# bebop/poly

Measured on AMD Instinct MI355X. Metric: mash.Sketch k-mers hashed/s, higher is better.
Workload: dtype u32

## Files before the change

### poly_amd/csrc/mash_sketch.hip

```cpp
#include <hip/hip_runtime.h>

#include <algorithm>

#include "common.h"
#include "host_pipeline.h"
#include "multi_device.h"
#include <memory>
#include <string>
#include <vector>

#ifndef PH_WPE
#define PH_WPE 6
#endif
#ifndef PH_CAPK
#define PH_CAPK 12u
#endif
#ifndef PH_ABL
#define PH_ABL 0
#endif
#ifndef PH_SEL_ATOMIC
#define PH_SEL_ATOMIC 0
#endif
#ifndef PH_BS_WIN
#define PH_BS_WIN 4
#endif
#ifndef PH_BS_U
#define PH_BS_U 4
#endif
#ifndef PH_SLAB_SIG
#define PH_SLAB_SIG 6u
#endif
#ifndef PH_SLAB_CW
#define PH_SLAB_CW 6u
#endif
#ifndef PH_SLAB_CF
#define PH_SLAB_CF 0u
#endif
#ifndef PH_SLAB_WPE
#define PH_SLAB_WPE 8
#endif

namespace polyhip {
namespace k1 {

constexpr int THREADS = 256;
constexpr int WAVES = THREADS / 64;
#ifndef PH_WTW
#define PH_WTW 512
#endif
constexpr int WTW = PH_WTW;
constexpr int TW = WTW * WAVES;
constexpr int GROUPS = WTW / (4 * 64);
constexpr int NB = 2048;
constexpr uint32_t MARK0 = 0xFFFFFFFFu, MARK1 = 0u;
constexpr int GBATCH = 32;
constexpr uint32_t WL_POSITIONAL = 0x80000000u;
constexpr uint32_t C1 = 0xcc9e2d51u, C2 = 0x1b873593u;

__device__ __forceinline__ uint32_t rotl32(uint32_t x, int r) { return (x << r) | (x >> (32 - r)); }

__device__ __forceinline__ uint32_t premix(uint32_t k)
{
    k *= C1;
    k = rotl32(k, 15);
    k *= C2;
    return k;
}

__device__ __forceinline__ uint32_t chain(uint32_t h) { return rotl32(h, 13) * 5u + 0xe6546b64u; }

__device__ __forceinline__ uint32_t fmix32(uint32_t h)
{
    h ^= h >> 16;
    h *= 0x85ebca6bu;
    h ^= h >> 13;
    h *= 0xc2b2ae35u;
    h ^= h >> 16;
    return h;
}

__device__ __forceinline__ uint32_t funnel_bytes(uint32_t hi, uint32_t lo, uint32_t sh)
{
    return __builtin_amdgcn_alignbyte(hi, lo, sh);
}

__device__ __forceinline__ uint32_t wave_incl_scan(uint32_t v)
{
    v += (uint32_t)__builtin_amdgcn_update_dpp(0, (int)v, 0x111, 0xF, 0xF, true);
    v += (uint32_t)__builtin_amdgcn_update_dpp(0, (int)v, 0x112, 0xF, 0xF, true);
    v += (uint32_t)__builtin_amdgcn_update_dpp(0, (int)v, 0x114, 0xF, 0xF, true);
    v += (uint32_t)__builtin_amdgcn_update_dpp(0, (int)v, 0x118, 0xF, 0xF, true);
    v += (uint32_t)__builtin_amdgcn_update_dpp(0, (int)v, 0x142, 0xA, 0xF, false);
    v += (uint32_t)__builtin_amdgcn_update_dpp(0, (int)v, 0x143, 0xC, 0xF, false);
    return v;
}

struct Smem {
    uint32_t *seqb;
    uint32_t *P;
    uint32_t *cand;
    uint32_t *binned;
    uint32_t *misc;
    uint32_t *lut;
    uint32_t *bins;
    uint32_t *biglist;
    uint32_t listcap;
};

constexpr uint32_t BIG_BIN = 32;
constexpr uint32_t BIG_LIST_CAP = 512;

template <class Bin, class Emit>
__device__ __attribute__((noinline)) void rank_big_bins(const uint32_t *__restrict__ binned, const Bin *__restrict__ bins,
                                              const uint32_t *__restrict__ biglist, uint32_t nbig, uint32_t s, Emit emit)
{
    const int lane = threadIdx.x & 63, wave = threadIdx.x >> 6;
    const uint64_t below = (1ull << lane) - 1ull;
    for (uint32_t q = wave; q < nbig; q += WAVES) {
        const uint32_t b = biglist[q];
        const uint32_t st = b ? bins[b - 1] : 0u, en = bins[b];
        uint32_t base = st, lastv = 0;
        bool first = true;
        while (base < s && base < en) {
            uint32_t m = 0xFFFFFFFFu;
            bool has = false;
            for (uint32_t x = st + lane; x < en; x += 64) {
                const uint32_t o = binned[x];
                if (first || o > lastv) {
                    m = min(m, o);
                    has = true;
                }
            }
            if (__ballot(has) == 0ull)
                break;
#pragma unroll
            for (int d = 32; d >= 1; d >>= 1)
                m = min(m, (uint32_t)__shfl_xor((int)m, d, 64));
            for (uint32_t x0 = st; x0 < en; x0 += 64) {
                const uint32_t x = x0 + lane;
                const bool eq = x < en && binned[x] == m;
                const uint64_t mask = __ballot(eq);
                const uint32_t pos = base + (uint32_t)__builtin_popcountll(mask & below);
                if (eq && pos < s)
                    emit(pos, m);
                base += (uint32_t)__builtin_popcountll(mask);
            }
            lastv = m;
            first = false;
        }
    }
}

template <class ForEach>
__device__ uint32_t bottom_s(const Smem &sm, uint32_t s, uint32_t tau, uint32_t binned_cap, bool keep_partial,
                             ForEach for_each)
{
    const int tid = threadIdx.x;
    uint32_t *bins = sm.P;
    const int sig = 32 - __builtin_clz(tau | 1u);
    const int shift = sig > 11 ? sig - 11 : 0;
    __syncthreads();
// ... 166 lines not shown
    const int tail = (int)(k & 3);
    const uint32_t tailmask = tail == 0 ? 0u : (0xFFFFFFFFu >> (32 - 8 * tail));

    {
        const int nq = (WTW >> 2) + nblk;
        for (int q = lane; q < (PH_ABL == 1 ? 0 : nq); q += 64) {
            const uint32_t d0 = seqb[q], d1 = seqb[q + 1];
            uint4 p;
            p.x = premix(d0);
            p.y = premix(funnel_bytes(d1, d0, 1));
            p.z = premix(funnel_bytes(d1, d0, 2));
            p.w = premix(funnel_bytes(d1, d0, 3));
            reinterpret_cast<uint4 *>(P)[q] = p;
        }
    }
    wave_sync();

    const uint4 *P4 = reinterpret_cast<const uint4 *>(P);
#pragma unroll
    for (int g = 0; g < GROUPS; ++g) {
        const int wq = lane + 64 * g;
        uint32_t h[4] = {0u, 0u, 0u, 0u};
        if (KS > 0) {
#pragma unroll
            for (int j = 0; j < (PH_ABL == 2 ? 1 : (KS >> 2)); ++j) {
                const uint4 p = P4[wq + j];
                h[0] = chain(h[0] ^ p.x);
                h[1] = chain(h[1] ^ p.y);
                h[2] = chain(h[2] ^ p.z);
                h[3] = chain(h[3] ^ p.w);
            }
        } else {
            for (int j = 0; j < nblk; ++j) {
                const uint4 p = P4[wq + j];
                h[0] = chain(h[0] ^ p.x);
                h[1] = chain(h[1] ^ p.y);
                h[2] = chain(h[2] ^ p.z);
                h[3] = chain(h[3] ^ p.w);
            }
        }
        if (PH_ABL == 3) {
        } else if (tail == 1) {
            const uint32_t tb = seqb[wq + nblk];
            h[0] ^= lut[tb & 0xFFu];
            h[1] ^= lut[(tb >> 8) & 0xFFu];
            h[2] ^= lut[(tb >> 16) & 0xFFu];
            h[3] ^= lut[tb >> 24];
        } else if (tail) {
            const uint32_t d0 = seqb[wq + nblk], d1 = seqb[wq + nblk + 1];
            h[0] ^= premix(d0 & tailmask) ^ k;
            h[1] ^= premix(funnel_bytes(d1, d0, 1) & tailmask) ^ k;
            h[2] ^= premix(funnel_bytes(d1, d0, 2) & tailmask) ^ k;
            h[3] ^= premix(funnel_bytes(d1, d0, 3) & tailmask) ^ k;
        } else {
#pragma unroll
            for (int c = 0; c < 4; ++c)
                h[c] ^= k;
        }
#pragma unroll
        for (int c = 0; c < 4; ++c)
            h[c] = PH_ABL == 3 ? h[c] : fmix32(h[c]);
        emit(4u * (uint32_t)wq, h);
    }
    wave_sync();
}

template <int KS, bool LOCKSTEP, class Before, class EmitFull, class EmitPart>
__device__ __forceinline__ void run_tiles(const Smem &sm, const uint32_t *__restrict__ gdw, uint32_t gsh,
                                          int64_t gbytes, int64_t nwin, uint32_t k, uint32_t n_seq_dw, uint32_t n_P_w,
                                          Before before, EmitFull emit_full, EmitPart emit_part)
{
    const int wave = threadIdx.x >> 6;
    uint32_t *seqb = sm.seqb + wave * n_seq_dw;
    uint32_t *P = sm.P + wave * n_P_w;
    const int64_t stage_bytes = (int64_t)n_seq_dw * 4 + 4;
    auto is_full = [&](int64_t t0) { return (nwin - t0) >= (int64_t)WTW && t0 + stage_bytes <= gbytes; };
    Stager<KS> st;
    const int64_t first = (int64_t)wave * WTW;
    if (first < nwin)
        st.load(gdw, gsh, gbytes, first, n_seq_dw, is_full(first));
    for (int64_t T0 = 0; T0 < nwin; T0 += TW) {
        if (LOCKSTEP)
            before(T0);
        const int64_t t0 = T0 + first;
        if (t0 >= nwin)
            continue;
        const bool full = is_full(t0);
        st.store(seqb, gdw, gsh, gbytes, t0, n_seq_dw, full);
        wave_sync();
        if (t0 + TW < nwin)
            st.load(gdw, gsh, gbytes, t0 + TW, n_seq_dw, is_full(t0 + TW));
        if (full) {
            tile_compute<KS>(seqb, P, sm.lut, k, [&](uint32_t w0, const uint32_t(&h)[4]) { emit_full(t0, w0, h, 4u); });
        } else {
            const uint32_t wl = (uint32_t)((nwin - t0) < (int64_t)WTW ? (nwin - t0) : (int64_t)WTW);
            tile_compute<KS>(seqb, P, sm.lut, k, [&](uint32_t w0, const uint32_t(&h)[4]) {
                emit_part(t0, w0, h, w0 >= wl ? 0u : (wl - w0 < 4u ? wl - w0 : 4u));
            });
        }
    }
}

__device__ __forceinline__ void append4(uint32_t *__restrict__ counter, uint32_t *__restrict__ cand, uint32_t cap,
                                        const uint32_t (&h)[4], uint32_t nvalid, uint32_t tau)
{
    bool a[4];
    uint64_t m[4];
    uint32_t cnt[4], total = 0;
#pragma unroll
    for (int c = 0; c < 4; ++c) {
        a[c] = (PH_ABL == 4 ? h[c] == 12345u : h[c] <= tau) && (uint32_t)c < nvalid;
        m[c] = __ballot(a[c]);
        cnt[c] = (uint32_t)__popcll(m[c]);
        total += cnt[c];
    }
    if (total == 0)
        return;
    uint32_t base = 0;
    if ((threadIdx.x & 63) == 0)
        base = atomicAdd(counter, total);
    base = __builtin_amdgcn_readfirstlane(base);
#pragma unroll
    for (int c = 0; c < 4; ++c) {
        if (a[c]) {
            const uint32_t idx = base + __builtin_amdgcn_mbcnt_hi((uint32_t)(m[c] >> 32),
                                                                  __builtin_amdgcn_mbcnt_lo((uint32_t)m[c], 0u));
            if (idx < cap)
                cand[idx] = h[c];
        }
        base += cnt[c];
    }
}

constexpr int BSU = PH_BS_U;
constexpr uint32_t BS_MARGIN = (PH_BS_WIN + 3u) & ~3u;
#define BS_SYNC()              \
    do {                       \
        if (PH_ABL != 21)      \
            __syncthreads();   \
    } while (0)
template <bool FIN>
__device__ void bottom_s_fast(const Smem &sm, uint32_t s, uint32_t tau, uint32_t C, uint32_t nbf_log2,
                              uint32_t *__restrict__ outp, const uint32_t *__restrict__ src, uint32_t first,
                              uint32_t step, uint32_t cnt)
{
    const int tid = threadIdx.x;
    auto fin = [](uint32_t h) { return FIN ? h ^ (h >> 16) : h; };
    uint32_t *bins = sm.bins;
    const uint16_t *bins16 = reinterpret_cast<const uint16_t *>(bins);
    const int sig = 32 - __builtin_clz(tau | 1u);
    const int shift = sig > (int)nbf_log2 ? sig - (int)nbf_log2 : 0;
    auto one = [](uint32_t b) { return 1u << ((b & 1u) << 4); };
    const bool wide = nbf_log2 == 11u;
    if (wide)
        reinterpret_cast<uint4 *>(bins)[tid] = make_uint4(0, 0, 0, 0);
    else
        reinterpret_cast<uint2 *>(bins)[tid] = make_uint2(0, 0);
    if (tid == 0)
        sm.misc[8] = 0;
    if (PH_BS_WIN) {
        if (tid < PH_BS_WIN)
            sm.binned[-1 - tid] = 0u;
        else if (tid < 2 * PH_BS_WIN)
            sm.binned[C + (uint32_t)tid - PH_BS_WIN] = 0xFFFFFFFFu;
    }
    BS_SYNC();
    for (uint32_t i0 = first; i0 < cnt; i0 += BSU * step) {
        uint32_t h[BSU];
#pragma unroll
        for (int u = 0; u < BSU; ++u)
            h[u] = i0 + u * step < cnt ? fin(src[i0 + u * step]) : 0u;
#pragma unroll
        for (int u = 0; u < BSU; ++u)
            if (i0 + u * step < cnt) {
                const uint32_t b = h[u] >> shift;
                atomicAdd(&bins[b >> 1], one(b));
            }
    }
    BS_SYNC();
    {
        uint32_t w[4];
        if (wide) {
            const uint4 t = reinterpret_cast<const uint4 *>(bins)[tid];
            w[0] = t.x, w[1] = t.y, w[2] = t.z, w[3] = t.w;
        } else {
            const uint2 t = reinterpret_cast<const uint2 *>(bins)[tid];
            w[0] = t.x, w[1] = t.y, w[2] = 0u, w[3] = 0u;
        }
        uint32_t c[8], sum = 0;
#pragma unroll
        for (int i = 0; i < 8; ++i) {
            c[i] = (w[i >> 1] >> (16 * (i & 1))) & 0xFFFFu;
            sum += c[i];
        }
        const uint32_t incl = wave_incl_scan(sum);
        if ((tid & 63) == 63)
            sm.misc[4 + (tid >> 6)] = incl;
        BS_SYNC();
        uint32_t run = incl - sum;
        for (int w8 = 0; w8 < (tid >> 6); ++w8)
            run += sm.misc[4 + w8];
        const uint32_t b0 = (uint32_t)tid << (wide ? 3 : 2);
#pragma unroll
        for (int i = 0; i < 4; ++i) {
            w[i] = run | ((run + c[2 * i]) << 16);
            run += c[2 * i] + c[2 * i + 1];
        }
        if (wide)
            reinterpret_cast<uint4 *>(bins)[tid] = make_uint4(w[0], w[1], w[2], w[3]);
        else
            reinterpret_cast<uint2 *>(bins)[tid] = make_uint2(w[0], w[1]);
        if (max(max(max(c[0], c[1]), max(c[2], c[3])), max(max(c[4], c[5]), max(c[6], c[7]))) > BIG_BIN) {
#pragma unroll
            for (int i = 0; i < 8; ++i)
                if (c[i] > BIG_BIN) {
                    const uint32_t slot = atomicAdd(&sm.misc[8], 1u);
                    if (slot < sm.listcap)
                        sm.biglist[slot] = b0 + (uint32_t)i;
                }
        }
    }
    BS_SYNC();
    for (uint32_t i0 = first; i0 < cnt; i0 += BSU * step) {
        uint32_t h[BSU], at[BSU];
#pragma unroll
        for (int u = 0; u < BSU; ++u)
            h[u] = i0 + u * step < cnt ? fin(src[i0 + u * step]) : 0u;
#pragma unroll
        for (int u = 0; u < BSU; ++u)
            if (i0 + u * step < cnt) {
                const uint32_t b = h[u] >> shift;
                at[u] = (atomicAdd(&bins[b >> 1], one(b)) >> ((b & 1u) << 4)) & 0xFFFFu;
            }
#pragma unroll
        for (int u = 0; u < BSU; ++u)
            if (i0 + u * step < cnt)
                sm.binned[at[u]] = h[u];
    }
    BS_SYNC();
    const uint32_t nbig = sm.misc[8];
    const bool by_waves = nbig <= sm.listcap;
    auto rank_in_bin = [&](uint32_t j, uint32_t hv) {
        const uint32_t b = hv >> shift;
        const uint32_t start = b ? bins16[b - 1] : 0u, end = bins16[b];
        if (start >= s || (by_waves && end - start > BIG_BIN))
            return;
        uint32_t pos = start;
        for (uint32_t x = start; x < end; ++x) {
            const uint32_t o = sm.binned[x];
            pos += (o < hv) || (o == hv && x < j);
        }
        if (pos < s)
            outp[pos] = hv;
    };
#if PH_BS_WIN
    if (PH_ABL != 22) {
        const uint32_t lim = 1u << shift;
        for (uint32_t j = tid; j < C; j += THREADS) {
            const uint32_t *__restrict__ w = sm.binned + j;
            const uint32_t hv = w[0];
            uint32_t pos = j;
            bool far;
            {
                uint32_t l[PH_BS_WIN], r[PH_BS_WIN];
#pragma unroll
                for (int d = 0; d < PH_BS_WIN; ++d) {
                    l[d] = w[-1 - d];
                    r[d] = w[1 + d];
                }
#pragma unroll
                for (int d = 0; d < PH_BS_WIN; ++d) {
                    pos -= l[d] > hv ? 1u : 0u;
                    pos += r[d] < hv ? 1u : 0u;
                }
                far = ((l[PH_BS_WIN - 1] ^ hv) < lim) | ((r[PH_BS_WIN - 1] ^ hv) < lim);
            }
            if (__builtin_expect(far, 0))
                rank_in_bin(j, hv);
            else if (pos < s)
                outp[pos] = hv;
        }
    }
#else
    for (uint32_t j = tid; j < C; j += THREADS)
        rank_in_bin(j, sm.binned[j]);
#endif
    if (by_waves && nbig)
        rank_big_bins(sm.binned, bins16, sm.biglist, nbig, s, [outp](uint32_t pos, uint32_t hv) { outp[pos] = hv; });
}

struct ReadView {
    const uint32_t *gdw;
    uint32_t gsh;
    int64_t gbytes, nwin;
};

__device__ __forceinline__ ReadView view(const uint8_t *__restrict__ seqs, const uint64_t *__restrict__ offs,
                                         uint64_t r, uint32_t k)
{
    ReadView v;
    const uint64_t o0 = offs[r], o1 = offs[r + 1];
    const int64_t n = (int64_t)(o1 - o0);
    v.nwin = n - (int64_t)k;
    v.gsh = (uint32_t)((uintptr_t)(seqs + o0) & 3);
    v.gdw = reinterpret_cast<const uint32_t *>(seqs + o0 - v.gsh);
    v.gbytes = n + v.gsh;
    return v;
}

template <int KS>
__global__ __launch_bounds__(THREADS) __attribute__((amdgpu_waves_per_eu(PH_WPE, 8))) void sketch_fast_kernel(const uint8_t *__restrict__ seqs,
                                                             const uint64_t *__restrict__ offs, uint64_t nseq,
                                                             uint32_t k_rt, uint32_t s, uint32_t *__restrict__ out,
                                                             uint32_t n_seq_dw, uint32_t n_P_w, uint32_t n_P,
                                                             uint32_t capf, uint32_t nbf_log2)
{
    extern __shared__ __attribute__((aligned(16))) uint32_t smem_raw[];
    Smem sm;
    sm.seqb = smem_raw;
    sm.P = sm.seqb + WAVES * n_seq_dw;
    sm.cand = sm.P + n_P;
    sm.binned = sm.cand + capf + BS_MARGIN;
    sm.misc = sm.binned + capf + BS_MARGIN;
    sm.lut = sm.misc + 16;
    sm.bins = sm.P;
    sm.biglist = sm.seqb;
    sm.listcap = BIG_LIST_CAP;

    const uint32_t k = KS > 0 ? (uint32_t)KS : k_rt;
    const int tid = threadIdx.x;
    sm.lut[tid] = premix((uint32_t)tid) ^ k;
    auto nothing = [](int64_t) {};

    for (uint64_t r = blockIdx.x; r < nseq; r += gridDim.x) {
        const ReadView rv = view(seqs, offs, r, k);
        if (rv.nwin <= 0)
            continue;
        uint32_t *__restrict__ outp = out + r * (uint64_t)s;

        if (rv.nwin < (int64_t)s) {
            __syncthreads();
            auto put = [&](int64_t t0, uint32_t w0, const uint32_t(&h)[4], uint32_t nvalid) {
#pragma unroll
                for (int c = 0; c < 4; ++c)
                    if ((uint32_t)c < nvalid)
                        outp[t0 + w0 + c] = h[c];
            };
            run_tiles<KS, false>(sm, rv.gdw, rv.gsh, rv.gbytes, rv.nwin, k, n_seq_dw, n_P_w, nothing, put, put);
            continue;
        }

        uint32_t tau0 = 0xFFFFFFFFu;
        {
            const uint64_t target = (uint64_t)s + 6ull * (uint64_t)__builtin_sqrtf((float)s) + 16ull;
            if ((int64_t)target < rv.nwin)
                tau0 = (uint32_t)((target << 32) / (uint64_t)rv.nwin);
        }
        bool ok = tau0 != 0xFFFFFFFFu || rv.nwin <= (int64_t)capf;
        __syncthreads();
        if (tid == 0)
            sm.misc[0] = 0;
        __syncthreads();
        uint32_t C = 0;
        if (ok) {
            auto keep = [&](int64_t, uint32_t, const uint32_t(&h)[4], uint32_t nvalid) {
                append4(&sm.misc[0], sm.cand, capf, h, nvalid, tau0);
            };
            run_tiles<KS, false>(sm, rv.gdw, rv.gsh, rv.gbytes, rv.nwin, k, n_seq_dw, n_P_w, nothing, keep, keep);
            __syncthreads();
            C = sm.misc[0];
            ok = C >= s && C <= capf;
        }
        if (ok) {
            if (PH_ABL == 5) {
                for (uint32_t i = tid; i < s; i += THREADS)
                    outp[i] = sm.cand[i];
            } else {
                bottom_s_fast<false>(sm, s, tau0, C, nbf_log2, outp, sm.cand, (uint32_t)tid, THREADS, C);
            }
        } else if (tid == 0) {
            outp[0] = MARK0;
            outp[1] = MARK1;
        }
    }
}

template <int KS> struct Slabs {
    static constexpr int NBLK = KS >> 2, TAIL = KS & 3;
    static constexpr int DUPD = NBLK + 2;
    const uint32_t *__restrict__ gdw;
    uint32_t gsh;
    uint32_t *__restrict__ seqb;
    uint32_t *__restrict__ P;
    const uint32_t *__restrict__ lut;
    int lane;

    uint32_t u_inside;
    uint32_t gb32;
    __device__ __forceinline__ void gload(uint32_t u, uint32_t &lo, uint32_t &hi) const
    {
        const uint32_t *__restrict__ slab = gdw + (uint64_t)u * 64;
        hi = 0u;
        if (__builtin_expect(u < u_inside, 1)) {
            lo = slab[lane];
            if (gsh)
                hi = slab[lane + 1];
        } else {
            const int left = (int)(gb32 - u * 256u);
            lo = lane * 4 < left ? slab[lane] : 0u;
            if (gsh)
                hi = (lane + 1) * 4 < left ? slab[lane + 1] : 0u;
        }
    }

    template <int PAR> __device__ __forceinline__ void stage(uint32_t lo, uint32_t hi) const
    {
        const uint32_t v = gsh ? funnel_bytes(hi, lo, gsh) : lo;
        seqb[1 + 64 * PAR + lane] = v;
        if (PAR == 0) {
            if (lane < DUPD)
                seqb[129 + lane] = v;
        } else if (lane == 63) {
            seqb[0] = v;
        }
    }

    template <int PAR> __device__ __forceinline__ void premix_unit() const
    {
        const uint32_t d0 = seqb[64 * PAR + lane], d1 = seqb[64 * PAR + lane + 1];
        uint4 p;
        p.x = premix(d0);
        p.y = premix(funnel_bytes(d1, d0, 1));
        p.z = premix(funnel_bytes(d1, d0, 2));
        p.w = premix(funnel_bytes(d1, d0, 3));
        uint4 *P4 = reinterpret_cast<uint4 *>(P);
        if (PAR == 0) {
            P4[(lane + 127) & 127] = p;
            if (lane >= 1 && lane <= NBLK)
                P4[127 + lane] = p;
        } else {
            P4[63 + lane] = p;
        }
    }

    template <int PAR> __device__ __forceinline__ void hash(uint32_t (&h)[4]) const
    {
        const uint4 *b = reinterpret_cast<const uint4 *>(P) + 64 * PAR + lane;
        h[0] = h[1] = h[2] = h[3] = 0u;
#pragma unroll
        for (int j = 0; j < (PH_ABL == 16 ? 1 : NBLK); ++j) {
            const uint4 p = b[j];
            h[0] = chain(h[0] ^ p.x);
            h[1] = chain(h[1] ^ p.y);
            h[2] = chain(h[2] ^ p.z);
            h[3] = chain(h[3] ^ p.w);
        }
        const uint32_t *t = seqb + 1 + 64 * PAR + lane + NBLK;
        if (TAIL == 1) {
            const uint32_t tb = t[0];
            uint32_t off[4];
            const uint32_t two = 2u;
            asm("v_lshlrev_b32_sdwa %0, %1, %2 dst_sel:DWORD dst_unused:UNUSED_PAD src0_sel:DWORD src1_sel:BYTE_0" : "=v"(off[0]) : "v"(two), "v"(tb));
            asm("v_lshlrev_b32_sdwa %0, %1, %2 dst_sel:DWORD dst_unused:UNUSED_PAD src0_sel:DWORD src1_sel:BYTE_1" : "=v"(off[1]) : "v"(two), "v"(tb));
            asm("v_lshlrev_b32_sdwa %0, %1, %2 dst_sel:DWORD dst_unused:UNUSED_PAD src0_sel:DWORD src1_sel:BYTE_2" : "=v"(off[2]) : "v"(two), "v"(tb));
            asm("v_lshlrev_b32_sdwa %0, %1, %2 dst_sel:DWORD dst_unused:UNUSED_PAD src0_sel:DWORD src1_sel:BYTE_3" : "=v"(off[3]) : "v"(two), "v"(tb));
#pragma unroll
            for (int c = 0; c < 4; ++c)
                h[c] ^= *reinterpret_cast<const __attribute__((address_space(3))) uint32_t *>((uintptr_t)off[c]);
        } else if (TAIL) {
            constexpr uint32_t tailmask = 0xFFFFFFFFu >> (32 - 8 * (TAIL ? TAIL : 1));
            const uint32_t d0 = t[0], d1 = t[1];
            h[0] ^= premix(d0 & tailmask) ^ (uint32_t)KS;
            h[1] ^= premix(funnel_bytes(d1, d0, 1) & tailmask) ^ (uint32_t)KS;
            h[2] ^= premix(funnel_bytes(d1, d0, 2) & tailmask) ^ (uint32_t)KS;
            h[3] ^= premix(funnel_bytes(d1, d0, 3) & tailmask) ^ (uint32_t)KS;
        } else {
#pragma unroll
            for (int c = 0; c < 4; ++c)
                h[c] ^= (uint32_t)KS;
        }
#pragma unroll
        for (int c = 0; c < 4; ++c) {
            uint32_t x = h[c];
            if (PH_ABL != 17) {
                x ^= x >> 16;
                x *= 0x85ebca6bu;
                x ^= x >> 13;
            }
            x *= 0xc2b2ae35u;
            h[c] = x;
        }
    }
};

template <bool PARTIAL>
__device__ __forceinline__ void append_own(uint32_t *__restrict__ seg, uint32_t capw, uint32_t &cnt, const uint32_t (&h)[4],
                                           uint32_t nvalid, uint32_t tauq)
{
    bool a[4];
    uint64_t m[4];
    uint32_t n[4], total = 0;
#pragma unroll
    for (int c = 0; c < 4; ++c) {
        a[c] = h[c] <= tauq && (!PARTIAL || (uint32_t)c < nvalid);
        m[c] = __ballot(a[c]);
        n[c] = (uint32_t)__popcll(m[c]);
        total += n[c];
    }
    uint32_t base = __builtin_amdgcn_readfirstlane(cnt);
    cnt = base + total;
#if PH_SEL_ATOMIC
    {
        uint32_t *ctr = seg + capw;
        uint32_t slot[4];
#pragma unroll
        for (int c = 0; c < 4; ++c)
            if (a[c])
                slot[c] = atomicInc(ctr, capw - 1u);
#pragma unroll
        for (int c = 0; c < 4; ++c)
            if (a[c])
                seg[slot[c]] = h[c];
        return;
    }
#endif
    if (cnt <= capw) {
#pragma unroll
        for (int c = 0; c < 4; ++c) {
            uint32_t *__restrict__ at = seg + base;
            if (a[c])
                at[__builtin_amdgcn_mbcnt_hi((uint32_t)(m[c] >> 32), __builtin_amdgcn_mbcnt_lo((uint32_t)m[c], 0u))] = h[c];
            base += n[c];
        }
    }
}

template <int KS>
__device__ __forceinline__ uint32_t run_slabs(const Smem &sm, const ReadView &rv, uint32_t n_seq_dw, uint32_t n_P_w,
                                              uint32_t *__restrict__ seg, uint32_t capw, uint32_t tauq)
{
    const int wave = __builtin_amdgcn_readfirstlane(threadIdx.x >> 6);
    Slabs<KS> S;
    S.gdw = rv.gdw;
    S.gsh = rv.gsh;
    S.seqb = sm.seqb + wave * n_seq_dw;
    S.P = sm.P + wave * n_P_w;
    S.lut = sm.lut;
    S.lane = threadIdx.x & 63;
    const uint32_t nslab = (uint32_t)((rv.nwin + 255) >> 8);
    const uint32_t spw = (nslab + WAVES - 1) / WAVES;
    const uint32_t a = (uint32_t)wave * spw, b = a + spw < nslab ? a + spw : nslab;
    S.u_inside = rv.gbytes >= 65 * 4 ? (uint32_t)(((rv.gbytes >> 2) - 65) >> 6) + 1u : 0u;
    S.gb32 = (uint32_t)rv.gbytes;
    const uint32_t nfull = (uint32_t)(rv.nwin >> 8), rem = (uint32_t)rv.nwin & 255u;
    uint32_t cnt = 0;
#if PH_SEL_ATOMIC
    capw -= 1u;
    if (S.lane == 0)
        seg[capw] = 0u;
#endif
    if (a >= b)
        return cnt;
    uint32_t l1, h1;
    S.gload(a, l1, h1);
    if (a & 1) {
        S.template stage<1>(l1, h1);
        wave_sync();
        S.gload(a + 1, l1, h1);
        S.template premix_unit<1>();
    } else {
        S.template stage<0>(l1, h1);
        wave_sync();
        S.gload(a + 1, l1, h1);
        S.template premix_unit<0>();
    }
    for (uint32_t i = a; i < b; ++i) {
        uint32_t h[4];
        if (i & 1) {
            S.template stage<0>(l1, h1);
            wave_sync();
            S.gload(i + 2, l1, h1);
            if (PH_ABL != 15)
                S.template premix_unit<0>();
            wave_sync();
            S.template hash<1>(h);
        } else {
            S.template stage<1>(l1, h1);
            wave_sync();
            S.gload(i + 2, l1, h1);
            if (PH_ABL != 15)
                S.template premix_unit<1>();
            wave_sync();
            S.template hash<0>(h);
        }
        if (PH_ABL == 11) {
            if ((h[0] ^ h[1] ^ h[2] ^ h[3]) == 0x12345u)
                seg[0] = h[0];
        } else if (__builtin_expect(i < nfull, 1)) {
            append_own<false>(seg, capw, cnt, h, 4u, tauq);
        } else {
            const int mine = (int)rem - 4 * S.lane;
            append_own<true>(seg, capw, cnt, h, mine <= 0 ? 0u : (mine < 4 ? (uint32_t)mine : 4u), tauq);
        }
        wave_sync();
    }
    return cnt;
}

template <int KS>
__global__ __launch_bounds__(THREADS) __attribute__((amdgpu_waves_per_eu(PH_SLAB_WPE, 8))) void sketch_slab_kernel(
    const uint8_t *__restrict__ seqs, const uint64_t *__restrict__ offs, uint64_t nseq, uint32_t s, uint32_t *__restrict__ out,
    uint32_t n_seq_dw, uint32_t n_P_w, uint32_t n_span, uint32_t capw, uint32_t capf, uint32_t nbf_log2)
{
    extern __shared__ __attribute__((aligned(16))) uint32_t smem_raw[];
    Smem sm;
    sm.lut = smem_raw;
    sm.seqb = smem_raw + 256;
    sm.P = sm.seqb + WAVES * n_seq_dw;
    sm.bins = sm.seqb;
    sm.binned = sm.bins + ((1u << nbf_log2) >> 1) + BS_MARGIN;
    sm.biglist = sm.binned + capf + BS_MARGIN;
    sm.listcap = (uint32_t)(sm.seqb + n_span - sm.biglist);
    sm.misc = sm.seqb + n_span;
    sm.cand = sm.misc + 16;
    constexpr uint32_t k = (uint32_t)KS;
    const int tid = threadIdx.x, wave = __builtin_amdgcn_readfirstlane(tid >> 6);
    sm.lut[tid] = premix((uint32_t)tid) ^ k;
    uint32_t *seg = sm.cand + wave * capw;

    for (uint64_t r = blockIdx.x; r < nseq; r += gridDim.x) {
        const ReadView rv = view(seqs, offs, r, k);
        if (rv.nwin <= 0)
            continue;
        uint32_t *__restrict__ outp = out + r * (uint64_t)s;
        if (rv.nwin < (int64_t)s)
            continue;
        uint32_t tauq = 0xFFFFFFFFu;
        {
            const uint64_t target = (uint64_t)s + (uint64_t)PH_SLAB_SIG * (uint64_t)__builtin_sqrtf((float)s) + 16ull;
            if ((int64_t)target < rv.nwin)
                tauq = (uint32_t)((target << 32) / (uint64_t)rv.nwin) | 0xFFFFu;
        }
        __syncthreads();
        const uint32_t cw = PH_ABL == 14 ? tauq >> 31 : run_slabs<KS>(sm, rv, n_seq_dw, n_P_w, seg, capw, tauq);
        if ((tid & 63) == 0)
            sm.misc[10 + wave] = cw;
        __syncthreads();
        if (PH_ABL == 11 || PH_ABL == 12 || PH_ABL == 14) {
            if (sm.misc[10] + sm.misc[11] + sm.misc[12] + sm.misc[13] == 0xFFFFFFF0u)
                outp[0] = cw;
            continue;
        }
        const uint32_t c0 = sm.misc[10], c1 = sm.misc[11], c2 = sm.misc[12], c3 = sm.misc[13];
        const uint32_t C = c0 + c1 + c2 + c3;
        const bool ok = max(max(c0, c1), max(c2, c3)) <= capw - (PH_SEL_ATOMIC ? 1u : 0u) && C >= s && C <= capf;
        if (ok)
            bottom_s_fast<true>(sm, s, tauq, C, nbf_log2, outp, seg, (uint32_t)(tid & 63), 64u, cw);
        else if (tid == 0) {
            outp[0] = MARK0;
            outp[1] = MARK1;
        }
    }
}

template <int KS>
__global__ __launch_bounds__(THREADS) void sketch_general_kernel(const uint8_t *__restrict__ seqs,
                                                                const uint64_t *__restrict__ offs, uint32_t k_rt,
                                                                uint32_t s, uint32_t *__restrict__ out,
                                                                uint32_t n_seq_dw, uint32_t n_P_w, uint32_t n_P,
                                                                uint32_t cap, uint64_t nseq, int take_positional)
{
    extern __shared__ __attribute__((aligned(16))) uint32_t smem_raw[];
    Smem sm;
    sm.seqb = smem_raw;
    sm.P = sm.seqb + WAVES * n_seq_dw;
    sm.cand = sm.P + n_P;
    sm.binned = sm.cand + cap;
    sm.misc = sm.binned + cap;
    sm.lut = sm.misc + 16;
    __shared__ uint32_t wl[GBATCH];
    __shared__ uint32_t nwl;

    const uint32_t k = KS > 0 ? (uint32_t)KS : k_rt;
    const int tid = threadIdx.x;
    sm.lut[tid] = premix((uint32_t)tid) ^ k;

    for (uint64_t base = (uint64_t)blockIdx.x * GBATCH; base < nseq; base += (uint64_t)gridDim.x * GBATCH) {
        __syncthreads();
        if (tid == 0)
            nwl = 0;
        __syncthreads();
        {
            const uint64_t r = base + tid;
            if (tid < GBATCH && r < nseq) {
                const int64_t nwin = (int64_t)(offs[r + 1] - offs[r]) - (int64_t)k;
                uint32_t need = 0;
                if (nwin >= (int64_t)s) {
                    const uint32_t *row = out + r * (uint64_t)s;
                    if (row[0] == MARK0 && row[1] == MARK1)
                        need = 1;
                } else if (nwin > 0 && take_positional) {
                    need = 2;
                }
                if (need)
                    wl[atomicAdd(&nwl, 1u)] = (uint32_t)tid | (need == 2 ? WL_POSITIONAL : 0u);
            }
        }
        __syncthreads();
        const uint32_t nredo = nwl;
    for (uint32_t q = 0; q < nredo; ++q) {
        const uint32_t entry = wl[q];
        const uint64_t r = base + (entry & ~WL_POSITIONAL);
        const ReadView rv = view(seqs, offs, r, k);
        uint32_t *__restrict__ outp = out + r * (uint64_t)s;
        __syncthreads();
        if (entry & WL_POSITIONAL) {
            auto put = [&](int64_t t0, uint32_t w0, const uint32_t(&h)[4], uint32_t nvalid) {
#pragma unroll
                for (int c = 0; c < 4; ++c)
                    if ((uint32_t)c < nvalid)
                        outp[t0 + w0 + c] = h[c];
            };
            run_tiles<KS, false>(sm, rv.gdw, rv.gsh, rv.gbytes, rv.nwin, k, n_seq_dw, n_P_w, [](int64_t) {}, put, put);
            continue;
        }
        if (tid == 0) {
            sm.misc[0] = 0;
            sm.misc[1] = 0xFFFFFFFFu;
        }
        __syncthreads();
        auto shrink_shared = [&]() {
            const uint32_t C = sm.misc[0];
            bottom_s(sm, s, sm.misc[1], cap, true, [&](auto f) {
                for (uint32_t i = tid; i < C; i += THREADS)
                    f(sm.cand[i]);
            });
        };
        auto append = [&](int64_t, uint32_t, const uint32_t(&h)[4], uint32_t nvalid) {
            append4(&sm.misc[0], sm.cand, cap, h, nvalid, sm.misc[1]);
        };
        run_tiles<KS, true>(
            sm, rv.gdw, rv.gsh, rv.gbytes, rv.nwin, k, n_seq_dw, n_P_w,
            [&](int64_t) {
                __syncthreads();
                const bool room = sm.misc[0] + (uint32_t)TW <= cap;
                __syncthreads();
                if (!room)
                    shrink_shared();
            },
            append, append);
        __syncthreads();
        shrink_shared();
        for (uint32_t i = tid; i < s; i += THREADS)
            outp[i] = sm.cand[i];
    }
    }
}


constexpr uint32_t WIDE_ROUND = 4 * THREADS;

__device__ __forceinline__ uint32_t murmur3_window(const uint8_t *__restrict__ p, uint32_t k)
{
    uint32_t h = 0;
    const uint32_t nblk = k >> 2;
    for (uint32_t j = 0; j < nblk; ++j) {
        uint32_t w;
        __builtin_memcpy(&w, p + 4 * (size_t)j, 4);
        h = chain(h ^ premix(w));
    }
    const uint8_t *t = p + 4 * (size_t)nblk;
    uint32_t w = 0;
    switch (k & 3u) {
    case 3: w ^= (uint32_t)t[2] << 16; [[fallthrough]];
    case 2: w ^= (uint32_t)t[1] << 8; [[fallthrough]];
    case 1: w ^= (uint32_t)t[0]; h ^= premix(w); break;
    default: break;
    }
    return fmix32(h ^ k);
}

__global__ __launch_bounds__(THREADS) void sketch_wide_kernel(const uint8_t *__restrict__ seqs,
                                                             const uint64_t *__restrict__ offs, uint64_t nseq, uint32_t k,
                                                             uint32_t s, uint32_t *__restrict__ out,
                                                             uint32_t *__restrict__ scratch, uint32_t cap)
{
    __shared__ uint32_t bins[NB];
    __shared__ uint32_t biglist[BIG_LIST_CAP];
    __shared__ uint32_t misc[16];
    Smem sm;
    sm.seqb = biglist;
    sm.P = bins;
    sm.cand = scratch + (size_t)blockIdx.x * 2 * cap;
    sm.binned = sm.cand + cap;
    sm.misc = misc;
    sm.lut = nullptr;
    const int tid = threadIdx.x;
    for (uint64_t r = blockIdx.x; r < nseq; r += gridDim.x) {
        const uint64_t o0 = offs[r];
        const int64_t nwin = (int64_t)(offs[r + 1] - o0) - (int64_t)k;
        if (nwin <= 0)
            continue;
        const uint8_t *__restrict__ sp = seqs + o0;
        uint32_t *__restrict__ outp = out + r * (uint64_t)s;
        if (nwin < (int64_t)s) {
            for (int64_t w = tid; w < nwin; w += THREADS)
                outp[w] = murmur3_window(sp + w, k);
            continue;
        }
        __syncthreads();
        if (tid == 0) {
            misc[0] = 0;
            misc[1] = 0xFFFFFFFFu;
        }
        __syncthreads();
        auto shrink = [&]() {
            const uint32_t C = misc[0];
            bottom_s(sm, s, misc[1], cap, true, [&](auto f) {
                for (uint32_t i = tid; i < C; i += THREADS)
                    f(sm.cand[i]);
            });
        };
        for (int64_t base = 0; base < nwin; base += WIDE_ROUND) {
            __syncthreads();
            const bool room = misc[0] + WIDE_ROUND <= cap;
            __syncthreads();
            if (!room)
                shrink();
            const uint32_t tau = misc[1];
#pragma unroll
            for (int c = 0; c < 4; ++c) {
                const int64_t w = base + c * THREADS + tid;
                if (w < nwin) {
                    const uint32_t h = murmur3_window(sp + w, k);
                    if (h <= tau)
                        sm.cand[atomicAdd(&misc[0], 1u)] = h;
                }
            }
        }
        __syncthreads();
        shrink();
        for (uint32_t i = tid; i < s; i += THREADS)
            outp[i] = sm.cand[i];
    }
}

__global__ __launch_bounds__(THREADS) void sketch_tiny_kernel(const uint8_t *__restrict__ seqs,
                                                             const uint64_t *__restrict__ offs, uint64_t nseq, uint32_t k,
                                                             uint32_t s, uint32_t *__restrict__ out,
                                                             unsigned long long *__restrict__ first_panic)
{
    const int tid = threadIdx.x;
    for (uint64_t r = blockIdx.x; r < nseq; r += gridDim.x) {
        const uint64_t o0 = offs[r];
        const int64_t nwin = (int64_t)(offs[r + 1] - o0) - (int64_t)k;
        if (nwin <= 0)
            continue;
        if (s == 0) {
            if (tid == 0)
                atomicMin(first_panic, (unsigned long long)r);
            continue;
        }
        const uint8_t *__restrict__ sp = seqs + o0;
        const uint32_t h0 = murmur3_window(sp, k);
        bool under = false;
        for (int64_t w = 1 + tid; w < nwin && !under; w += THREADS)
            under = murmur3_window(sp + w, k) < h0;
        if (__syncthreads_or(under ? 1 : 0)) {
            if (tid == 0)
                atomicMin(first_panic, (unsigned long long)r);
        } else if (tid == 0) {
            out[r] = h0;
        }
    }
}

struct Launch {
    uint32_t n_seq_dw, n_P_w, n_P, n_P_fast, nbf_log2, nbf_log2_slab, capf, cap, capw, capf_slab, n_span;
    size_t smem_fast, smem_general, smem_slab;
};

static Launch plan(uint32_t k, uint32_t s)
{
    Launch L;
    const uint32_t nblk = k / 4;
    L.n_seq_dw = ((WTW / 4 + nblk + 2) + 3u) & ~3u;
    L.n_P_w = WTW + 4 * nblk;
    L.n_P = WAVES * L.n_P_w;
    L.n_P_fast = L.n_P < 1024u ? 1024u : L.n_P;
    L.nbf_log2 = L.n_P_fast >= 2048u ? 11u : 10u;
    if (L.n_P < (uint32_t)NB)
        L.n_P = NB;
    const uint32_t s4 = (s + 3u) & ~3u;
    uint32_t rt = 1;
    while ((uint64_t)rt * rt < s)
        ++rt;
    L.capf = (s4 + PH_CAPK * rt + 64u + 63u) & ~63u;
    L.cap = s4 + TW + 64u;
    const size_t common = (size_t)WAVES * L.n_seq_dw + L.n_P + 16 + 256;
    L.smem_fast = ((size_t)WAVES * L.n_seq_dw + L.n_P_fast + 16 + 256 + 2 * (size_t)L.capf + 2 * BS_MARGIN) * 4;
    if (PH_ABL == 7)
        L.smem_fast = 70 * 1024;
    L.smem_general = (common + 2 * (size_t)L.cap) * 4;
    {
        const uint32_t target = s + PH_SLAB_SIG * rt + 16u;
        const uint32_t exp_w = (target + WAVES - 1) / WAVES;
        uint32_t rw = 1;
        while ((uint64_t)rw * rw < exp_w)
            ++rw;
        L.capw = (exp_w + PH_SLAB_CW * rw + 8u + 63u) & ~63u;
        L.capf_slab = PH_SLAB_CF ? ((target + PH_SLAB_CF * rt + 8u + 63u) & ~63u) : L.capf;
    }
    L.nbf_log2_slab = 11;
    {
        const uint32_t rings = WAVES * (L.n_seq_dw + L.n_P_w);
        const uint32_t sorted = ((1u << L.nbf_log2_slab) >> 1) + L.capf_slab + 2 * BS_MARGIN + L.capf_slab / (BIG_BIN + 1) + 1;
        L.n_span = rings > sorted ? rings : sorted;
    }
    L.smem_slab = ((size_t)256 + L.n_span + 16 + (size_t)WAVES * L.capw) * 4;
#ifdef PH_LDS_PAD
    L.smem_slab += PH_LDS_PAD;
#endif
    return L;
}

static unsigned persistent_grid(size_t smem, uint64_t n)
{
    const uint64_t per_cu = std::max<uint64_t>(1, std::min<uint64_t>(8, (160 * 1024) / std::max<size_t>(smem, 1)));
    return (unsigned)std::min<uint64_t>(n, 256 * per_cu * 4);
}

template <int KS>
static int launch(const uint8_t *d_seqs, const uint64_t *d_offs, uint64_t n, uint32_t k, uint32_t s,
                  uint32_t *d_out, const Launch &L, hipStream_t st)
{
    auto general = sketch_general_kernel<KS>;
    PH_HIP(hipFuncSetAttribute(reinterpret_cast<const void *>(general), hipFuncAttributeMaxDynamicSharedMemorySize,
                               (int)L.smem_general));
    bool slabs = false;
    if constexpr (KS > 0) {
        slabs = !env_is("POLYHIP_K1_SLABS", '0') && L.smem_slab <= 64 * 1024;
        if (slabs) {
            auto slab = sketch_slab_kernel<KS>;
            PH_HIP(hipFuncSetAttribute(reinterpret_cast<const void *>(slab), hipFuncAttributeMaxDynamicSharedMemorySize,
                                       (int)L.smem_slab));
            hipLaunchKernelGGL(slab, dim3(persistent_grid(L.smem_slab, n)), dim3(THREADS), L.smem_slab, st, d_seqs, d_offs, n, s,
                               d_out, L.n_seq_dw, L.n_P_w, L.n_span, L.capw, L.capf_slab, L.nbf_log2_slab);
        }
    }
    if (!slabs) {
        auto fast = sketch_fast_kernel<KS>;
        PH_HIP(hipFuncSetAttribute(reinterpret_cast<const void *>(fast), hipFuncAttributeMaxDynamicSharedMemorySize,
                                   (int)L.smem_fast));
        hipLaunchKernelGGL(fast, dim3(persistent_grid(L.smem_fast, n)), dim3(THREADS), L.smem_fast, st, d_seqs, d_offs, n,
                           k, s, d_out, L.n_seq_dw, L.n_P_w, L.n_P_fast, L.capf, L.nbf_log2);
    }
    PH_HIP(hipGetLastError());
    const unsigned ggrid = (unsigned)std::min<uint64_t>((n + GBATCH - 1) / GBATCH, persistent_grid(L.smem_general, n));
    hipLaunchKernelGGL(general, dim3(ggrid), dim3(THREADS), L.smem_general, st, d_seqs, d_offs, k, s, d_out, L.n_seq_dw,
                       L.n_P_w, L.n_P, L.cap, n, slabs ? 1 : 0);
    PH_HIP(hipGetLastError());
    return POLYHIP_OK;
}

}
}

using namespace polyhip;

extern "C" {

int polyhip_mash_sketch_batch_dev(const uint8_t *d_seqs, const uint64_t *d_offsets, uint64_t n, uint32_t k,
                                  uint32_t s, uint32_t *d_out, polyhip_stream_t stream)
{
    if (n == 0)
        return POLYHIP_OK;
    PH_REQUIRE(d_seqs && d_offsets && (d_out || s == 0), "polyhip_mash_sketch_batch: null pointer");
    PH_REQUIRE(s <= (1u << 24), "polyhip_mash_sketch_batch: SketchSize %u > 2^24 is not implemented", s);
    hipStream_t st = as_stream(stream);
    if (s < 2) {
        unsigned long long *d_first = nullptr, h_first = ~0ull;
        PH_HIP(hipMallocAsync(reinterpret_cast<void **>(&d_first), sizeof h_first, st));
        StreamFree guard{d_first, st};
        PH_HIP(hipMemsetAsync(d_first, 0xFF, sizeof h_first, st));
        hipLaunchKernelGGL(k1::sketch_tiny_kernel, dim3((unsigned)std::min<uint64_t>(n, 4096)), dim3(k1::THREADS), 0, st, d_seqs,
                           d_offsets, n, k, s, d_out, d_first);
        PH_HIP(hipGetLastError());
        PH_HIP(hipMemcpyAsync(&h_first, d_first, sizeof h_first, hipMemcpyDeviceToHost, st));
        PH_HIP(guard.release());
        PH_HIP(hipStreamSynchronize(st));
        if (h_first != ~0ull)
            return set_error(POLYHIP_ERR_PANIC,
                             "mash.Sketch with SketchSize %u indexes Sketches[-1] on sequence %llu (mash.go:%s): the reference panics",
                             s, h_first + (unsigned long long)md::base().item, s == 0 ? "96" : "98");
        return POLYHIP_OK;
    }
    const k1::Launch L = k1::plan(k <= 4096 ? k : 4096, s <= 8192 ? s : 8192);
    if (s > 8192 || k > 4096 || L.smem_general > 160 * 1024) {
        const uint32_t s4 = (s + 3u) & ~3u;
        const uint32_t cap = 2 * s4 + 2 * k1::WIDE_ROUND;
        const uint64_t per_wg = 2ull * cap * sizeof(uint32_t), budget = 4ull << 30;
        const unsigned grid = (unsigned)std::max<uint64_t>(
            1, std::min<uint64_t>(std::min<uint64_t>(n, s > 16384 ? 256 : 1024), budget / per_wg));
        uint32_t *scratch = nullptr;
        PH_HIP(hipMallocAsync(reinterpret_cast<void **>(&scratch), (size_t)grid * per_wg, st));
        StreamFree guard{scratch, st};
        hipLaunchKernelGGL(k1::sketch_wide_kernel, dim3(grid), dim3(k1::THREADS), 0, st, d_seqs, d_offsets, n, k, s, d_out, scratch,
                           cap);
        PH_HIP(hipGetLastError());
        PH_HIP(guard.release());
        return POLYHIP_OK;
    }
    const uint64_t CHUNK = 1ull << 30;
    for (uint64_t i0 = 0; i0 < n; i0 += CHUNK) {
        const uint64_t m = n - i0 < CHUNK ? n - i0 : CHUNK;
        const uint64_t *offs = d_offsets + i0;
        uint32_t *outp = d_out + i0 * (uint64_t)s;
        int rc;
        switch (k) {
        case 17: rc = k1::launch<17>(d_seqs, offs, m, k, s, outp, L, st); break;
        case 21: rc = k1::launch<21>(d_seqs, offs, m, k, s, outp, L, st); break;
        case 31: rc = k1::launch<31>(d_seqs, offs, m, k, s, outp, L, st); break;
        default: rc = k1::launch<0>(d_seqs, offs, m, k, s, outp, L, st); break;
        }
        if (rc != POLYHIP_OK)
            return rc;
    }
    return POLYHIP_OK;
}

static int sketch_batch_one(const uint8_t *seqs, const uint64_t *offsets, uint64_t n, uint32_t k, uint32_t s, uint32_t *out)
{
    if (n == 0)
        return POLYHIP_OK;
    PH_REQUIRE(seqs && offsets && (out || s == 0), "polyhip_mash_sketch_batch: null pointer");
    PH_REQUIRE(s <= (1u << 24), "polyhip_mash_sketch_batch: SketchSize %u > 2^24 is not implemented", s);
    bool need_prior = false;
    for (uint64_t i = 0; i < n; ++i) {
        PH_REQUIRE(offsets[i] <= offsets[i + 1], "polyhip_mash_sketch_batch: offsets not ascending at %llu",
                   (unsigned long long)(i + md::base().item));
        need_prior |= offsets[i + 1] - offsets[i] < (uint64_t)k + s;
    }
    const uint64_t CHUNK = 256ull << 20, row = (uint64_t)s * sizeof(uint32_t);
    std::vector<uint64_t> cut{0};
    uint64_t max_bytes = 0, max_reads = 0;
    for (uint64_t i = 0; i < n;) {
        uint64_t j = i, sz = 0;
        do {
            sz += offsets[j + 1] - offsets[j] + row;
            ++j;
        } while (j < n && sz < CHUNK);
        cut.push_back(j);
        max_bytes = std::max(max_bytes, offsets[j] - offsets[i]);
        max_reads = std::max(max_reads, j - i);
        i = j;
    }
    struct Slot {
        DevBuf dseq, doff, dout;
        hipStream_t st = nullptr;
        hipEvent_t computed = nullptr;
        std::vector<uint64_t> hoff;
        ~Slot()
        {
            if (st) {
                (void)hipStreamSynchronize(st);
                (void)hipStreamDestroy(st);
            }
            if (computed)
                (void)hipEventDestroy(computed);
        }
    } slot[2];
    struct DlStream {
        hipStream_t s = nullptr;
        ~DlStream()
        {
            if (s) {
                (void)hipStreamSynchronize(s);
                (void)hipStreamDestroy(s);
            }
        }
    } dls;
    const size_t nchunks = cut.size() - 1;
    int first_panic = POLYHIP_OK;
    std::string panic_text;
    for (size_t q = 0; q < std::min<size_t>(2, nchunks); ++q) {
        PH_HIP(slot[q].dseq.alloc(max_bytes + 16));
        PH_HIP(slot[q].doff.alloc((max_reads + 1) * sizeof(uint64_t)));
        PH_HIP(slot[q].dout.alloc(max_reads * row));
        PH_HIP(hipStreamCreateWithFlags(&slot[q].st, hipStreamNonBlocking));
        PH_HIP(hipEventCreateWithFlags(&slot[q].computed, hipEventDisableTiming));
        slot[q].hoff.resize(max_reads + 1);
    }
    PH_HIP(hipStreamCreateWithFlags(&dls.s, hipStreamNonBlocking));
    int dev = 0;
// ... 93 lines not shown
```

Before: 845.7 billion.

## Specialize slab main loop, mask LDS appends, and cut bottom-s ranking range

Splits the slab hashing loop into a specialized interior path with unconditional loads and a compile-time shift flag, plus a generic tail. Candidate appends now use one inline-asm sequence of exec-masked ds_write ops. Bottom-s ranking stops at the end of the bin holding the s-th element rather than scanning all C candidates. tauq is computed with 32-bit division, and the slab path is disabled when s >= 32768. Together these aim to cut per-k-mer instruction overhead and wasted ranking work. The cost is fragile inline asm, and the early cutoff reads binned[s-1] before ranking, which looks like it assumes the array is already sorted at that point.

New measurement: 870.7 billion, median of 6. +2.9%, better.

```diff
diff --git a/poly_amd/csrc/k1_tauq.h b/poly_amd/csrc/k1_tauq.h
--- /dev/null
+++ b/poly_amd/csrc/k1_tauq.h
@@ -0,0 +1,23 @@
+#pragma once
+#include <cstdint>
+
+#if defined(__HIPCC__)
+#define PH_TAUQ_HD __host__ __device__
+#else
+#define PH_TAUQ_HD
+#endif
+
+namespace polyhip {
+namespace k1 {
+
+PH_TAUQ_HD inline uint32_t slab_tauq(uint32_t target, int64_t nwin)
+{
+    if ((int64_t)target >= nwin)
+        return 0xFFFFFFFFu;
+    if (nwin >= ((int64_t)1 << 32))
+        return 0xFFFFu;
+    return (((target << 16) / (uint32_t)nwin) << 16) | 0xFFFFu;
+}
+
+}
+}
diff --git a/poly_amd/csrc/mash_sketch.hip b/poly_amd/csrc/mash_sketch.hip
--- a/poly_amd/csrc/mash_sketch.hip
+++ b/poly_amd/csrc/mash_sketch.hip
@@ -3,10 +3,12 @@
 #include <algorithm>
 
 #include "common.h"
+#include "k1_tauq.h"
 #include "host_pipeline.h"
 #include "multi_device.h"
 #include <memory>
 #include <string>
+#include <type_traits>
 #include <vector>
 
 #ifndef PH_WPE
@@ -479,10 +481,12 @@
     const int shift = sig > (int)nbf_log2 ? sig - (int)nbf_log2 : 0;
     auto one = [](uint32_t b) { return 1u << ((b & 1u) << 4); };
     const bool wide = nbf_log2 == 11u;
+    uint32_t z;
+    asm volatile("v_mov_b32 %0, 0" : "=v"(z));
     if (wide)
-        reinterpret_cast<uint4 *>(bins)[tid] = make_uint4(0, 0, 0, 0);
+        reinterpret_cast<uint4 *>(bins)[tid] = make_uint4(z, z, z, z);
     else
-        reinterpret_cast<uint2 *>(bins)[tid] = make_uint2(0, 0);
+        reinterpret_cast<uint2 *>(bins)[tid] = make_uint2(z, z);
     if (tid == 0)
         sm.misc[8] = 0;
     if (PH_BS_WIN) {
@@ -580,10 +584,11 @@
         if (pos < s)
             outp[pos] = hv;
     };
+    const uint32_t e_star = bins16[sm.binned[s - 1] >> shift];
 #if PH_BS_WIN
     if (PH_ABL != 22) {
         const uint32_t lim = 1u << shift;
-        for (uint32_t j = tid; j < C; j += THREADS) {
+        for (uint32_t j = tid; j < e_star; j += THREADS) {
             const uint32_t *__restrict__ w = sm.binned + j;
             const uint32_t hv = w[0];
             uint32_t pos = j;
@@ -609,7 +614,7 @@
         }
     }
 #else
-    for (uint32_t j = tid; j < C; j += THREADS)
+    for (uint32_t j = tid; j < e_star; j += THREADS)
         rank_in_bin(j, sm.binned[j]);
 #endif
     if (by_waves && nbig)
@@ -724,6 +729,15 @@
 
     uint32_t u_inside;
     uint32_t gb32;
+    template <bool SH> __device__ __forceinline__ void gload_inside(uint32_t u, uint32_t &lo, uint32_t &hi) const
+    {
+        const uint32_t *__restrict__ slab = gdw + (uint64_t)u * 64;
+        uint32_t off = (uint32_t)lane * 4u;
+        asm volatile("" : "+v"(off));
+        const uint8_t *__restrict__ p = reinterpret_cast<const uint8_t *>(slab) + off;
+        lo = *reinterpret_cast<const uint32_t *>(p);
+        hi = SH ? *reinterpret_cast<const uint32_t *>(p + 4) : 0u;
+    }
     __device__ __forceinline__ void gload(uint32_t u, uint32_t &lo, uint32_t &hi) const
     {
         const uint32_t *__restrict__ slab = gdw + (uint64_t)u * 64;
@@ -740,9 +754,9 @@
         }
     }
 
-    template <int PAR> __device__ __forceinline__ void stage(uint32_t lo, uint32_t hi) const
+    template <int PAR, bool SH = true> __device__ __forceinline__ void stage(uint32_t lo, uint32_t hi) const
     {
-        const uint32_t v = gsh ? funnel_bytes(hi, lo, gsh) : lo;
+        const uint32_t v = SH ? funnel_bytes(hi, lo, gsh) : lo;
         seqb[1 + 64 * PAR + lane] = v;
         if (PAR == 0) {
             if (lane < DUPD)
@@ -820,6 +834,30 @@
     }
 };
 
+__device__ __forceinline__ uint32_t lds_addr(const uint32_t *p)
+{
+    return (uint32_t)(uintptr_t)(const __attribute__((address_space(3))) uint32_t *)p;
+}
+
+__device__ __forceinline__ void lds_store4_masked(const uint32_t (&addr)[4], const uint32_t (&v)[4], const uint64_t (&mask)[4])
+{
+    uint64_t saved;
+    asm volatile("s_mov_b64 %0, exec\n\t"
+                 "s_mov_b64 exec, %9\n\t"
+                 "ds_write_b32 %1, %5\n\t"
+                 "s_mov_b64 exec, %10\n\t"
+                 "ds_write_b32 %2, %6\n\t"
+                 "s_mov_b64 exec, %11\n\t"
+                 "ds_write_b32 %3, %7\n\t"
+                 "s_mov_b64 exec, %12\n\t"
+                 "ds_write_b32 %4, %8\n\t"
+                 "s_mov_b64 exec, %0"
+                 : "=&s"(saved)
+                 : "v"(addr[0]), "v"(addr[1]), "v"(addr[2]), "v"(addr[3]), "v"(v[0]), "v"(v[1]), "v"(v[2]), "v"(v[3]),
+                   "s"(mask[0]), "s"(mask[1]), "s"(mask[2]), "s"(mask[3])
+                 : "memory");
+}
+
 template <bool PARTIAL>
 __device__ __forceinline__ void append_own(uint32_t *__restrict__ seg, uint32_t capw, uint32_t &cnt, const uint32_t (&h)[4],
                                            uint32_t nvalid, uint32_t tauq)
@@ -834,7 +872,7 @@
         n[c] = (uint32_t)__popcll(m[c]);
         total += n[c];
     }
-    uint32_t base = __builtin_amdgcn_readfirstlane(cnt);
+    uint32_t base = cnt;
     cnt = base + total;
 #if PH_SEL_ATOMIC
     {
@@ -852,13 +890,14 @@
     }
 #endif
     if (cnt <= capw) {
+        uint32_t at[4];
 #pragma unroll
         for (int c = 0; c < 4; ++c) {
-            uint32_t *__restrict__ at = seg + base;
-            if (a[c])
-                at[__builtin_amdgcn_mbcnt_hi((uint32_t)(m[c] >> 32), __builtin_amdgcn_mbcnt_lo((uint32_t)m[c], 0u))] = h[c];
+            at[c] = lds_addr(seg + base) +
+                    4u * __builtin_amdgcn_mbcnt_hi((uint32_t)(m[c] >> 32), __builtin_amdgcn_mbcnt_lo((uint32_t)m[c], 0u));
             base += n[c];
         }
+        lds_store4_masked(at, h, m);
     }
 }
 
@@ -901,35 +940,58 @@
         S.gload(a + 1, l1, h1);
         S.template premix_unit<0>();
     }
-    for (uint32_t i = a; i < b; ++i) {
+    auto step = [&](auto par, auto main, auto sh, uint32_t i) {
+        constexpr int P = decltype(par)::value;
+        constexpr bool MAIN = decltype(main)::value, SH = decltype(sh)::value;
         uint32_t h[4];
-        if (i & 1) {
-            S.template stage<0>(l1, h1);
-            wave_sync();
+        S.template stage<1 - P, SH>(l1, h1);
+        wave_sync();
+        if (MAIN)
+            S.template gload_inside<SH>(i + 2, l1, h1);
+        else
             S.gload(i + 2, l1, h1);
-            if (PH_ABL != 15)
-                S.template premix_unit<0>();
-            wave_sync();
-            S.template hash<1>(h);
-        } else {
-            S.template stage<1>(l1, h1);
-            wave_sync();
-            S.gload(i + 2, l1, h1);
-            if (PH_ABL != 15)
-                S.template premix_unit<1>();
-            wave_sync();
-            S.template hash<0>(h);
-        }
+        if (PH_ABL != 15)
+            S.template premix_unit<1 - P>();
+        wave_sync();
+        S.template hash<P>(h);
         if (PH_ABL == 11) {
             if ((h[0] ^ h[1] ^ h[2] ^ h[3]) == 0x12345u)
                 seg[0] = h[0];
-        } else if (__builtin_expect(i < nfull, 1)) {
+        } else if (MAIN || __builtin_expect(i < nfull, 1)) {
             append_own<false>(seg, capw, cnt, h, 4u, tauq);
         } else {
             const int mine = (int)rem - 4 * S.lane;
             append_own<true>(seg, capw, cnt, h, mine <= 0 ? 0u : (mine < 4 ? (uint32_t)mine : 4u), tauq);
         }
         wave_sync();
+    };
+    using P0 = std::integral_constant<int, 0>;
+    using P1 = std::integral_constant<int, 1>;
+    using T = std::true_type;
+    using F = std::false_type;
+    const uint32_t lim = nfull < b ? nfull : b;
+    const uint32_t ins = S.u_inside >= 2u ? S.u_inside - 2u : 0u;
+    const uint32_t m = ins < lim ? ins : lim;
+    uint32_t i = a;
+    auto main_loop = [&](auto sh) {
+        if ((i & 1) && i < m)
+            step(P1{}, T{}, sh, i++);
+        for (; i + 1 < m; i += 2) {
+            step(P0{}, T{}, sh, i);
+            step(P1{}, T{}, sh, i + 1);
+        }
+        if (i < m)
+            step(P0{}, T{}, sh, i++);
+    };
+    if (S.gsh)
+        main_loop(T{});
+    else
+        main_loop(F{});
+    for (; i < b; ++i) {
+        if (i & 1)
+            step(P1{}, F{}, T{}, i);
+        else
+            step(P0{}, F{}, T{}, i);
     }
     return cnt;
 }
@@ -962,12 +1024,7 @@
         uint32_t *__restrict__ outp = out + r * (uint64_t)s;
         if (rv.nwin < (int64_t)s)
             continue;
-        uint32_t tauq = 0xFFFFFFFFu;
-        {
-            const uint64_t target = (uint64_t)s + (uint64_t)PH_SLAB_SIG * (uint64_t)__builtin_sqrtf((float)s) + 16ull;
-            if ((int64_t)target < rv.nwin)
-                tauq = (uint32_t)((target << 32) / (uint64_t)rv.nwin) | 0xFFFFu;
-        }
+        const uint32_t tauq = slab_tauq(s + PH_SLAB_SIG * (uint32_t)__builtin_sqrtf((float)s) + 16u, rv.nwin);
         __syncthreads();
         const uint32_t cw = PH_ABL == 14 ? tauq >> 31 : run_slabs<KS>(sm, rv, n_seq_dw, n_P_w, seg, capw, tauq);
         if ((tid & 63) == 0)
@@ -1266,7 +1323,7 @@
                                (int)L.smem_general));
     bool slabs = false;
     if constexpr (KS > 0) {
-        slabs = !env_is("POLYHIP_K1_SLABS", '0') && L.smem_slab <= 64 * 1024;
+        slabs = !env_is("POLYHIP_K1_SLABS", '0') && L.smem_slab <= 64 * 1024 && s < 32768u;
         if (slabs) {
             auto slab = sketch_slab_kernel<KS>;
             PH_HIP(hipFuncSetAttribute(reinterpret_cast<const void *>(slab), hipFuncAttributeMaxDynamicSharedMemorySize,
```
